# dtee1/reinforcement-learning-for-playing-tetris-with-prescribed-initial-configuration-and-limited-moves

Hardware: AMD Instinct MI355X
Metric: env-steps/sec (whole node) at 1M parallel 20x10 boards (higher is better)
Workload: dtype u32

## Files before the change

### reinforcement-learning-for-playing-tetris-with-prescribed-initial-configuration-and-limited-moves_amd/csrc/tetris_piclim.hip

```cpp
#include "tpl_internal.h"
#include "tpl_observe.h"
#include "tpl_step.h"

#include <hip/hip_bf16.h>

#include <type_traits>

#include <cstdarg>
#include <cstdio>
#include <cstring>
#include <new>

namespace tpl {

static thread_local char g_err[512] = "";

int fail_msg(int code, const char* fmt, ...) {
    va_list ap;
    va_start(ap, fmt);
    vsnprintf(g_err, sizeof(g_err), fmt, ap);
    va_end(ap);
    return code;
}

static inline size_t align_up(size_t x, size_t a) { return (x + a - 1) / a * a; }
constexpr size_t kPlanePad = 512 * 4;
static inline size_t plane_bytes(int64_t n) { return align_up((size_t)n, kPlanePad) * sizeof(uint4); }
static inline size_t clock_bytes(int64_t n) { return align_up((size_t)n, kPlanePad) / kClockGroup * sizeof(unsigned long long); }
static inline int piece_words(int M) { return M / kWindowStride + 1; }
static inline uint32_t record_stride_shift(int M) {
    const size_t need = 32 + 8 * (size_t)(piece_words(M) - 1);
    uint32_t shift = 6;
    while (((size_t)1 << shift) < need) ++shift;
    return shift;
}
static inline size_t record_stride(int M) { return (size_t)1 << record_stride_shift(M); }

#ifdef TPL_DIAG_CLOCK
#define TPL_STAMP(k) stamp[k] = __builtin_amdgcn_s_memrealtime()
#else
#define TPL_STAMP(k) do { } while (0)
#endif

template <bool kActionForm, bool kAutoReset, int kBpl, int kThreads, typename Obs = void>
__global__ __launch_bounds__(kThreads) void step_kernel(const StepArgs p) {
    constexpr bool kObserve = !std::is_void<Obs>::value;
    static_assert(!kObserve || kBpl == 1, "step-and-observe: one board per lane");
    static_assert((int)sizeof(uint32_t) * kLdsCols * kLdsStride <= obs::kWaveLds, "the column words fit the wave's observation bytes");
    __shared__ ShapeWord s_shape[32];
    __shared__ uint32_t s_stat[4];
    __shared__ uint32_t s_cols[kObserve ? 1 : kThreads / 64][kObserve ? 1 : kLdsCols][kObserve ? 1 : kLdsStride];
    __shared__ __attribute__((aligned(16))) uint8_t s_rows[kObserve ? kThreads / 64 : 1][kObserve ? obs::kWaveLds : 16];
#ifdef TPL_DIAG_CLOCK
    unsigned long long stamp[6] = {0, 0, 0, 0, 0, 0};
#endif
    TPL_STAMP(0);

    const int64_t base = (int64_t)blockIdx.x * (kThreads * kBpl) + threadIdx.x;
    uint4 A[kBpl], B[kBpl];
    uint32_t a0[kBpl], a1[kBpl];
    unsigned long long clock[kBpl];
    bool valid[kBpl];
#pragma unroll
    for (int k = 0; k < kBpl; ++k) {
        const int64_t i = base + (int64_t)k * kThreads;
        valid[k] = i < p.n;
        const int64_t j = valid[k] ? i : p.n - 1;
        A[k] = p.plane_a[i];
        B[k] = p.plane_b[i];
        const int64_t wave_first = (int64_t)blockIdx.x * (kThreads * kBpl) + (int64_t)k * kThreads +
                                   (int64_t)(__builtin_amdgcn_readfirstlane((int)threadIdx.x) & ~63);
        clock[k] = p.clock[wave_first >> kClockShift];
        a0[k] = load_int<true>(p.act0, p.int_shift, j);
        a1[k] = kActionForm ? 0u : load_int<true>(p.act1, p.int_shift, j);
    }
    if (threadIdx.x < 32) s_shape[threadIdx.x] = kShapeTable[threadIdx.x];
    if (threadIdx.x < 4) s_stat[threadIdx.x] = 0;
    __syncthreads();

    uint64_t word[kBpl];
    uint32_t moves[kBpl], refill_word[kBpl];
    bool live[kBpl], refill[kBpl];
#pragma unroll
    for (int k = 0; k < kBpl; ++k) {
        asm volatile("" ::"v"(A[k].x), "v"(B[k].x), "v"(a0[k]), "v"(a1[k]), "s"(clock[k]));
    }
    TPL_STAMP(1);
    __builtin_amdgcn_s_setprio(3);
#pragma unroll
    for (int k = 0; k < kBpl; ++k) {
        moves[k] = packed_moves(A[k]);
        const uint32_t tenth = tenths(moves[k] + 1u);
        refill_word[k] = window_word(tenth);
        live[k] = packed_state(B[k]) == ST_RUNNING;
        refill[k] = live[k] && window_runs_out(tenth) && (p.n_cfg[0] | p.n_cfg[1]) != 0u;
    }
#pragma unroll
    for (int k = 0; k < kBpl; ++k) {
        const int64_t i = base + (int64_t)k * kThreads;
        word[k] = 0;
        if (refill[k]) {
            const uint32_t slot = packed_slot(B[k]);
            const uint32_t cfg = config_of(p, (uint32_t)i, clock[k] - moves[k], slot);
            word[k] = piece_word_at(pool_record(p, slot, cfg), refill_word[k]);
        }
    }

    float reward[kBpl];
    uint32_t n_clear[kBpl];
    bool done[kBpl], reload[kBpl];
#pragma unroll
    for (int k = 0; k < kBpl; ++k) {
        reward[k] = 0.0f;
        n_clear[k] = 0;
        done[k] = true;
        reload[k] = false;
        if (!live[k]) continue;
        uint32_t rot, loc;
        if (kActionForm) {
            split_action(a0[k], rot, loc);
        } else {
            rot = a0[k];
            loc = a1[k];
        }
        Board s;
        bool topout;
        unpack_board<true>(A[k], B[k], s);
        uint32_t* cols = kObserve ? (uint32_t*)s_rows[threadIdx.x >> 6] + (threadIdx.x & 63)
                                  : &s_cols[threadIdx.x >> 6][0][threadIdx.x & 63];
        lds_store_cols(cols, s.c);
        if (k == 0) {
#pragma unroll
            for (int c = kCols; c < kLdsCols; ++c) cols[c * kLdsStride] = kSentinelBit;
        }
        n_clear[k] = move_board_lds(s, cols, s_shape, rot, loc, p.L, p.M, topout);
        lds_load_cols(cols, s.c);
        next_window(s, refill[k], word[k]);

        reward[k] = step_reward(p, n_clear[k], s.state);
        done[k] = s.state != ST_RUNNING;
        if (done[k]) {
            atomicAdd(&s_stat[0], 1u);
            if (s.lines) atomicAdd(&s_stat[1], s.lines);
            if (s.state == ST_WON) atomicAdd(&s_stat[2], 1u);
            if (s.state == ST_LOST_TOPOUT) atomicAdd(&s_stat[3], 1u);
        }
        reload[k] = kAutoReset && done[k];
        pack_board<true>(s, A[k], B[k]);
    }

    TPL_STAMP(2);
#pragma unroll
    for (int k = 0; k < kBpl; ++k) {
        const int64_t i = base + (int64_t)k * kThreads;
        if (!valid[k]) continue;
        if (p.reward) p.reward[i] = reward[k];
        if (p.done) p.done[i] = done[k] ? 1 : 0;
        if (p.cleared) p.cleared[i] = (uint8_t)n_clear[k];
    }

    if (kAutoReset) {
        bool any = false;
#pragma unroll
        for (int k = 0; k < kBpl; ++k) any = any || reload[k];
        if (any) {
            uint4 RA[kBpl], RB[kBpl];
#pragma unroll
            for (int k = 0; k < kBpl; ++k) {
                const int64_t i = base + (int64_t)k * kThreads;
                const uint32_t cfg = config_of(p, (uint32_t)i, clock[k] + 1u, p.cur_slot);
                const uint4* rec = (const uint4*)pool_record(p, p.cur_slot, reload[k] ? cfg : 0u);
                RA[k] = rec[0];
                RB[k] = rec[1];
            }
#pragma unroll
            for (int k = 0; k < kBpl; ++k) {
                if (!reload[k]) continue;
                A[k] = RA[k];
                B[k] = make_uint4(RB[k].x, RB[k].y | (p.cur_slot << 30), RB[k].z, RB[k].w);
            }
        }
    }

#ifdef TPL_DIAG_CLOCK
#pragma unroll
    for (int k = 0; k < kBpl; ++k) asm volatile("" ::"v"(A[k].x), "v"(B[k].x));
#endif
    TPL_STAMP(3);
#pragma unroll
    for (int k = 0; k < kBpl; ++k) {
        const int64_t i = base + (int64_t)k * kThreads;
        if (!kAutoReset && !live[k]) continue;
        p.plane_a[i] = A[k];
        p.plane_b[i] = B[k];
    }
    if constexpr (kBpl % 2 == 0) {
        static_assert(kBpl == 2 || kBpl == 4, "one call of store_pair per two boards of a lane");
        const int lane = threadIdx.x & 63;
        const int64_t group_first = (int64_t)blockIdx.x * (kThreads * kBpl) + (threadIdx.x & ~63) + ((lane >> 4) & 1) * kClockGroup;
        const auto store_pair = [&](int k, unsigned long long even, unsigned long long odd) {
            const int64_t i = group_first + (int64_t)(k + (lane >> 5)) * kThreads;
            p.clock[i >> kClockShift] = (lane >> 5 ? odd : even) + 1u;
        };
        store_pair(0, clock[0], clock[1]);
        if constexpr (kBpl == 4) store_pair(2, clock[2], clock[3]);
    } else {
#pragma unroll
        for (int k = 0; k < kBpl; ++k) {
            const int64_t i = base + (int64_t)k * kThreads;
            p.clock[i >> kClockShift] = clock[k] + 1u;
        }
    }

    TPL_STAMP(4);
    if constexpr (kObserve) {
        const int lane = threadIdx.x & 63;
        const int64_t wave_base = (int64_t)blockIdx.x * kThreads + (threadIdx.x & ~63);
        const int64_t left = p.n - wave_base;
        const int count = left >= 64 ? 64 : left > 0 ? (int)left : 0;
        uint8_t* const rows = s_rows[threadIdx.x >> 6];
        int lines_left = 0;
        if (lane < count) {
            Board s;
            unpack_board(A[0], B[0], s);
            lines_left = obs::board_to_bytes(s, p.L, p.M, rows, lane);
        }
        if (count > 0) obs::store_span<Obs>(rows, lane, count, wave_base, lines_left, (Obs*)p.obs);
    }
    __syncthreads();
    if (s_stat[0] != 0) {
        if (threadIdx.x < 4) {
            const uint32_t v = s_stat[threadIdx.x];
            if (v) atomicAdd(&p.stats[(size_t)(blockIdx.x % kStatShards) * kStatStride + threadIdx.x],
                             (unsigned long long)v);
        }
    }
#ifdef TPL_DIAG_CLOCK
    __builtin_amdgcn_s_waitcnt(0);
    TPL_STAMP(5);
    if (p.diag && (threadIdx.x & 63) == 0) {
        unsigned long long* d = p.diag + 6 * ((size_t)blockIdx.x * (kThreads / 64) + (threadIdx.x >> 6));
        for (int k = 0; k < 6; ++k) d[k] = stamp[k];
    }
#endif
}

struct RolloutArgs {
    StepArgs s;
    const uint8_t* actions;
    uint64_t random_seed;
    uint32_t step0;
    uint8_t* actions_out;
    int64_t action_stride;
    uint32_t K;
    float* reward_steps;
    uint8_t* done_steps;
    float* reward_sum;
    uint32_t* finished;
    uint32_t* trajectory;
};

template <bool kAutoReset, bool kRandom, bool kCompact>
__global__ __launch_bounds__(kBlock) void rollout_kernel(const RolloutArgs q) {
    const StepArgs& p = q.s;
    __shared__ ShapeWord s_shape[32];
    __shared__ uint32_t s_stat[4];
    __shared__ uint32_t s_cols[kBlock / 64][kLdsCols][kLdsStride];
    const int64_t i = (int64_t)blockIdx.x * kBlock + threadIdx.x;
    const bool valid = i < p.n;
    uint4 A = make_uint4(0, 0, 0, 0), B = A;
    uint32_t act = 0;
    unsigned long long clock = 0;
    if (valid) {
        A = p.plane_a[i];
        B = p.plane_b[i];
        if (!kRandom) act = q.actions[i];
    }
    const int64_t wave_first = (int64_t)blockIdx.x * kBlock + (int64_t)(__builtin_amdgcn_readfirstlane((int)threadIdx.x) & ~63);
    if (wave_first < p.n) clock = p.clock[wave_first >> kClockShift];
    if (threadIdx.x < 32) s_shape[threadIdx.x] = kShapeTable[threadIdx.x];
    if (threadIdx.x < 4) s_stat[threadIdx.x] = 0;
    __syncthreads();

    RareTally tally;
    if (valid) {
        Board s;
        unpack_board<true>(A, B, s);
        uint32_t* cols = &s_cols[threadIdx.x >> 6][0][threadIdx.x & 63];
        lds_store_cols(cols, s.c);
#pragma unroll
        for (int k = kCols; k < kLdsCols; ++k) cols[k * kLdsStride] = kSentinelBit;
        const uint8_t* next_word = next_piece_word(current_record(s, p, (uint32_t)i, clock), s.moves);
        uint32_t until_refill = moves_until_refill(s.moves);
        const uint32_t draw_base = kRandom ? explore_base(q.random_seed, (uint64_t)(p.global_offset + i)) : 0u;
        uint32_t draw_pair = 0;
        float rsum = 0.0f;
        const int64_t block_first = (int64_t)blockIdx.x * kBlock;
        const uint32_t in_block = threadIdx.x;
        const uint8_t* act_row = q.actions + block_first;
        uint8_t* act_out_row = q.actions_out + block_first;
        float* reward_row = q.reward_steps + block_first;
        uint8_t* done_row = q.done_steps + block_first;
        const bool want_reward = !kCompact && q.reward_steps != nullptr, want_done = !kCompact && q.done_steps != nullptr;
        uint32_t* traj_row = q.trajectory + block_first;
        uint32_t traj_word = 0;
        asm volatile("" ::"v"(act));
        float reward_prev = 0.0f;
        bool done_prev = false;
        for (uint32_t k = 0; k < q.K; ++k) {
            if (!kCompact && k > 0) {
                if (want_reward) { __builtin_nontemporal_store(reward_prev, reward_row + in_block); reward_row += p.n; }
                if (want_done) { __builtin_nontemporal_store((uint8_t)(done_prev ? 1 : 0), done_row + in_block); done_row += p.n; }
            }
            if (kCompact && k > 0 && (k & 3u) == 0u) {
                __builtin_nontemporal_store(traj_word, traj_row + in_block);
                traj_row += p.n;
                traj_word = 0;
            }
            uint32_t act_next = 0;
            if (kRandom) {
                const uint32_t step = q.step0 + k;
                if (k == 0 || (step & 1u) == 0u) draw_pair = explore_pair(draw_base, q.random_seed, step);
                act = explore_pick(draw_pair, step);
                if (q.actions_out) { act_out_row[in_block] = (uint8_t)act; act_out_row += p.n; }
            } else {
                act_row += q.action_stride;
                if (k + 1 < q.K) act_next = act_row[in_block];
            }
            uint32_t rot, loc;
            split_small_action(act, rot, loc);
            float reward;
            uint32_t code;
            const bool done = advance_board_lds<kAutoReset>(s, cols, next_word, until_refill, rot, loc, p, (uint32_t)i, clock + k,
                                                            s_shape, reward, code, tally);
            if (kCompact) traj_word |= code << (8u * (k & 3u));
            else {
                rsum = rsum + reward;
                reward_prev = reward;
                done_prev = done;
            }
            act = act_next;
        }
        if (want_reward) __builtin_nontemporal_store(reward_prev, reward_row + in_block);
        if (want_done) __builtin_nontemporal_store((uint8_t)(done_prev ? 1 : 0), done_row + in_block);
        if (kCompact) __builtin_nontemporal_store(traj_word, traj_row + in_block);
        lds_load_cols(cols, s.c);
        pack_board<true>(s, A, B);
        p.plane_a[i] = A;
        p.plane_b[i] = B;
        if ((threadIdx.x & (kClockGroup - 1)) == 0) p.clock[i >> kClockShift] = clock + q.K;
        if (!kCompact && q.reward_sum) q.reward_sum[i] = rsum;
        if (q.finished) q.finished[i] = tally.episodes;
    }
    flush_tally(tally, s_stat, p.stats);
}

__global__ __launch_bounds__(kBlock) void reset_kernel(const StepArgs p, const uint8_t* mask) {
    const int64_t i = (int64_t)blockIdx.x * kBlock + threadIdx.x;
    if (i >= p.n) return;
    unsigned long long birth = 0;
    if (mask) {
        if (!mask[i]) return;
        birth = p.clock[i >> kClockShift];
    }
    const uint32_t cfg = config_of(p, (uint32_t)i, birth, p.cur_slot);
    uint4 A, B;
    load_config(p, cfg, A, B);
    p.plane_a[i] = A;
    p.plane_b[i] = B;
}

__device__ __forceinline__ uint64_t piece_word(const uint8_t* pc, uint32_t M, uint32_t w) {
    uint64_t word = 0;
    for (uint32_t j = 0; j < (uint32_t)kWindowEntries; ++j) {
        const uint32_t idx = w * kWindowStride + j;
        word |= (uint64_t)(idx <= M ? (uint32_t)(pc[idx] & 7u) : 7u) << (3u * j);
    }
    return word;
}

__global__ __launch_bounds__(kBlock) void pack_configs_kernel(const uint16_t* rows, const uint8_t* pieces, int64_t n_cfg,
                                                             uint32_t M, uint32_t words, uint8_t* pool, uint32_t stride) {
    const int64_t i = (int64_t)blockIdx.x * kBlock + threadIdx.x;
    if (i >= n_cfg) return;
    uint16_t r[kRows];
#pragma unroll
    for (int k = 0; k < kRows; ++k) r[k] = rows[i * kRows + k];
    Board s;
    rows_to_cols(r, s.c);
    const uint8_t* pc = pieces + (size_t)i * (M + 1);
    set_window(s, piece_word(pc, M, 0));
    s.state = ST_RUNNING; s.lines = 0; s.moves = 0; s.slot = 0;
    uint4 A, B;
    pack_board(s, A, B);
    uint8_t* rec = pool + (size_t)i * stride;
    ((uint4*)rec)[0] = A;
    ((uint4*)rec)[1] = B;
    for (uint32_t w = 1; w < words; ++w) ((uint64_t*)(rec + 32))[w - 1] = piece_word(pc, M, w);
}

__global__ __launch_bounds__(kBlock) void build_side_kernel(const uint8_t* pool, uint32_t stride_shift, int64_t n_cfg, uint8_t* side) {
    const int64_t i = (int64_t)blockIdx.x * kBlock + threadIdx.x;
    if (i >= n_cfg) return;
    const uint4* rec = (const uint4*)(pool + ((size_t)i << stride_shift));
    Board s;
    unpack_board<true>(rec[0], rec[1], s);
    uint4* sr = (uint4*)(side + ((size_t)i << kSideShift));
    sr[0] = make_uint4(s.c[0], s.c[1], s.c[2], s.c[3]);
    sr[1] = make_uint4(s.c[4], s.c[5], s.c[6], s.c[7]);
    sr[2] = make_uint4(s.c[8], s.c[9], s.window, s.window_hi);
    sr[3] = make_uint4(0, 0, 0, 0);
}

__global__ __launch_bounds__(kBlock) void export_kernel(const uint4* plane_a, const uint4* plane_b, int64_t n, uint32_t M,
                                                       uint16_t* rows, uint8_t* cur, uint8_t* nxt, uint8_t* lines,
                                                       uint8_t* moves, uint8_t* state, uint8_t* pieces_left) {
    const int64_t i = (int64_t)blockIdx.x * kBlock + threadIdx.x;
    if (i >= n) return;
    Board s;
    unpack_board(plane_a[i], plane_b[i], s);
    if (rows) {
#pragma unroll
        for (int r = 0; r < kRows; ++r) rows[i * kRows + r] = (uint16_t)row_of_cols(s.c, r);
    }
    if (cur) cur[i] = (uint8_t)(s.window & 7u);
    if (nxt) nxt[i] = (uint8_t)((s.window >> 3) & 7u);
    if (lines) lines[i] = (uint8_t)s.lines;
    if (moves) moves[i] = (uint8_t)s.moves;
    if (state) state[i] = (uint8_t)(s.state == ST_LOST_TOPOUT ? ST_LOST_LIMIT : s.state);
    if (pieces_left) pieces_left[i] = (uint8_t)(M + 1u - s.moves - (s.state == ST_LOST_TOPOUT ? 1u : 0u));
}

template <typename T>
__device__ __forceinline__ T obs_cast(float v);
template <> __device__ __forceinline__ float obs_cast<float>(float v) { return v; }
template <> __device__ __forceinline__ __hip_bfloat16 obs_cast<__hip_bfloat16>(float v) { return __float2bfloat16(v); }

template <typename T>
__global__ __launch_bounds__(kBlock) void expand_obs_kernel(const uint4* plane_a, const uint4* plane_b, int64_t n,
                                                           uint32_t L, uint32_t M, T* out) {
    __shared__ uint32_t s_bits[kBlock / 64][64][9];
    const int lane = threadIdx.x & 63;
    const int wave = threadIdx.x >> 6;
    const int64_t base = ((int64_t)blockIdx.x * (kBlock / 64) + wave) * 64;
    const int64_t i = base + lane;
    if (i < n) {
        Board s;
        unpack_board(plane_a[i], plane_b[i], s);
        uint32_t words[7] = {0, 0, 0, 0, 0, 0, 0};
#pragma unroll
        for (int r = 0; r < kRows; ++r) {
            const uint32_t row = row_of_cols(s.c, r);
            const int bit = r * 10;
            words[bit >> 5] |= row << (bit & 31);
            if ((bit & 31) > 22) words[(bit >> 5) + 1] |= row >> (32 - (bit & 31));
        }
#pragma unroll
        for (int k = 0; k < 7; ++k) s_bits[wave][lane][k] = words[k];
        const uint32_t terminal = s.state != ST_RUNNING ? 1u : 0u;
        s_bits[wave][lane][7] = (s.window & 63u) | (terminal << 6) | (s.lines << 8) | (s.moves << 16);
    }
    __syncthreads();
    const int64_t count = (n - base) < 64 ? (n - base) : 64;
    for (int64_t j = 0; j < count; ++j) {
        const uint32_t* bits = s_bits[wave][j];
        T* o = out + (base + j) * TPL_OBS_DIM;
        const uint32_t f = bits[7];
#pragma unroll
        for (int t = 0; t < 4; ++t) {
            const int e = lane + 64 * t;
            if (e < 200) {
                o[e] = obs_cast<T>((float)((bits[e >> 5] >> (e & 31)) & 1u));
            } else if (e < TPL_OBS_DIM) {
                float v;
                if (e < 207) v = ((f & 7u) == (uint32_t)(e - 200)) ? 1.0f : 0.0f;
                else if (e < 214) v = (((f >> 3) & 7u) == (uint32_t)(e - 207)) ? 1.0f : 0.0f;
                else if (e == 214) v = (float)((int)L - (int)((f >> 8) & 0xFFu));
                else if (e == 215) v = (float)((int)M - (int)((f >> 16) & 0xFFu));
                else v = (float)((f >> 6) & 1u);
                o[e] = obs_cast<T>(v);
            }
        }
// ... 670 lines not shown
```

### reinforcement-learning-for-playing-tetris-with-prescribed-initial-configuration-and-limited-moves_amd/csrc/tpl_device.h

```cpp
#pragma once

#include <hip/hip_runtime.h>
#include <stdint.h>

namespace tpl {

constexpr int kRows = 20;
constexpr int kCols = 10;
constexpr uint32_t kColMask = 0xFFFFFu;
constexpr int kWindowStride = 10;
constexpr int kWindowEntries = 12;
constexpr int kSideShift = 6;
constexpr int kClockGroup = 32;
constexpr int kClockShift = 5;

enum : uint32_t { ST_RUNNING = 0, ST_WON = 1, ST_LOST_LIMIT = 2, ST_LOST_TOPOUT = 3 };

struct Board {
    uint32_t c[kCols];
    uint32_t window;
    uint32_t window_hi;
    uint32_t state, lines, moves, slot;
};

__device__ __forceinline__ void set_window(Board& s, uint64_t word) {
    s.window = (uint32_t)word;
    s.window_hi = (uint32_t)(word >> 32) & 0xFu;
}
__device__ __forceinline__ void next_window(Board& s, bool refill, uint64_t word) {
    const uint32_t lo = __builtin_amdgcn_alignbit(s.window_hi, s.window, 3);
    const uint32_t hi = s.window_hi >> 3;
    s.window = refill ? (uint32_t)word : lo;
    s.window_hi = refill ? ((uint32_t)(word >> 32) & 0xFu) : hi;
}
__device__ __forceinline__ uint32_t tenths(uint32_t cursor) { return __umul24(cursor, 205u); }
__device__ __forceinline__ bool window_runs_out(uint32_t t) { return (t & 2047u) < 205u; }
__device__ __forceinline__ uint32_t window_word(uint32_t t) { return t >> 11; }

struct ShapeWord { uint32_t x, y; };

__host__ __device__ constexpr ShapeWord make_shape(int h, int w, int m0, int m1, int m2, int m3,
                                                   int t0, int t1, int t2, int t3) {
    const int m[4] = {m0, m1, m2, m3};
    const int t[4] = {t0, t1, t2, t3};
    uint32_t x = 0, y = 0;
    for (int c = 0; c < 4; ++c) {
        uint32_t colbits = 0;
        for (int i = 0; i < 4; ++i) colbits |= (uint32_t)((m[i] >> c) & 1) << i;
        x |= colbits << (4 * c);
        y |= (uint32_t)(c < w ? 3 - t[c] : 64) << (8 * c);
    }
    x |= (uint32_t)w << 16 | (uint32_t)h << 19 | (uint32_t)(kCols - w) << 22 | ((1u << h) - 1u) << 26;
    return ShapeWord{x, y};
}

#define TPL_I0 make_shape(1, 4, 15, 0, 0, 0, 0, 0, 0, 0)
#define TPL_I1 make_shape(4, 1, 1, 1, 1, 1, 3, 0, 0, 0)
#define TPL_L0 make_shape(2, 3, 4, 7, 0, 0, 1, 1, 1, 0)
#define TPL_L1 make_shape(3, 2, 3, 2, 2, 0, 0, 2, 0, 0)
#define TPL_L2 make_shape(2, 3, 7, 1, 0, 0, 1, 0, 0, 0)
#define TPL_L3 make_shape(3, 2, 1, 1, 3, 0, 2, 2, 0, 0)
#define TPL_J0 make_shape(2, 3, 1, 7, 0, 0, 1, 1, 1, 0)
#define TPL_J1 make_shape(3, 2, 2, 2, 3, 0, 2, 2, 0, 0)
#define TPL_J2 make_shape(2, 3, 7, 4, 0, 0, 0, 0, 1, 0)
#define TPL_J3 make_shape(3, 2, 3, 1, 1, 0, 2, 0, 0, 0)
#define TPL_T0 make_shape(2, 3, 2, 7, 0, 0, 1, 1, 1, 0)
#define TPL_T1 make_shape(3, 2, 2, 3, 2, 0, 1, 2, 0, 0)
#define TPL_T2 make_shape(2, 3, 7, 2, 0, 0, 0, 1, 0, 0)
#define TPL_T3 make_shape(3, 2, 1, 3, 1, 0, 2, 1, 0, 0)
#define TPL_S0 make_shape(2, 3, 6, 3, 0, 0, 1, 1, 0, 0)
#define TPL_S1 make_shape(3, 2, 1, 3, 2, 0, 1, 2, 0, 0)
#define TPL_Z0 make_shape(2, 3, 3, 6, 0, 0, 0, 1, 1, 0)
#define TPL_Z1 make_shape(3, 2, 2, 3, 1, 0, 2, 1, 0, 0)
#define TPL_O0 make_shape(2, 2, 3, 3, 0, 0, 1, 1, 0, 0)

#define TPL_SHAPE_LIST                                                                                    \
    TPL_I0, TPL_I1, TPL_I0, TPL_I1, TPL_L0, TPL_L1, TPL_L2, TPL_L3, TPL_J0, TPL_J1, TPL_J2, TPL_J3, TPL_T0,  \
    TPL_T1, TPL_T2, TPL_T3, TPL_S0, TPL_S1, TPL_S0, TPL_S1, TPL_Z0, TPL_Z1, TPL_Z0, TPL_Z1, TPL_O0, TPL_O0,  \
    TPL_O0, TPL_O0, TPL_O0, TPL_O0, TPL_O0, TPL_O0
__device__ __constant__ const ShapeWord kShapeTable[32] = {TPL_SHAPE_LIST};
constexpr ShapeWord kShapeTableHost[32] = {TPL_SHAPE_LIST};

__device__ __forceinline__ void pack3(uint32_t a, uint32_t b, uint32_t c, uint32_t& lo, uint32_t& hi) {
    lo = a | (b << 20);
    hi = (b >> 12) | (c << 8);
}

constexpr uint32_t kSentinelBit = 1u << kRows;

__device__ __forceinline__ uint32_t opaque_sgpr(uint32_t v) {
    uint32_t r;
    asm("s_mov_b32 %0, %1" : "=s"(r) : "i"(v));
    return r;
}

template <bool kSentinel>
__device__ __forceinline__ void unpack3(uint32_t lo, uint32_t hi, uint32_t& a, uint32_t& b, uint32_t& c) {
    if (kSentinel) {
        const uint32_t m = opaque_sgpr(kColMask), top = opaque_sgpr(kSentinelBit);
        a = (m & lo) | (~m & top);
        b = (m & __builtin_amdgcn_alignbit(hi, lo, 20)) | (~m & top);
        c = (m & (hi >> 8)) | (~m & top);
    } else {
        a = lo & kColMask;
        b = __builtin_amdgcn_alignbit(hi, lo, 20) & kColMask;
        c = (hi >> 8) & kColMask;
    }
}

template <bool kSentinel = false>
__device__ __forceinline__ void unpack_board(const uint4& A, const uint4& B, Board& s) {
    unpack3<kSentinel>(A.x, A.y, s.c[0], s.c[1], s.c[2]);
    unpack3<kSentinel>(A.z, A.w, s.c[3], s.c[4], s.c[5]);
    unpack3<kSentinel>(B.x, B.y, s.c[6], s.c[7], s.c[8]);
    if (kSentinel) {
        const uint32_t m = opaque_sgpr(kColMask), top = opaque_sgpr(kSentinelBit);
        s.c[9] = (m & B.z) | (~m & top);
    } else {
        s.c[9] = B.z & kColMask;
    }
    s.lines = (B.z >> 20) & 0xFFu;
    s.moves = (A.y >> 28) | ((A.w >> 28) << 4);
    s.window = B.w;
    s.window_hi = B.z >> 28;
    s.state = (B.y >> 28) & 3u;
    s.slot = (B.y >> 30) & 1u;
}

__device__ __forceinline__ uint32_t packed_state(const uint4& B) { return (B.y >> 28) & 3u; }
__device__ __forceinline__ uint32_t packed_slot(const uint4& B) { return (B.y >> 30) & 1u; }
__device__ __forceinline__ uint32_t packed_moves(const uint4& A) { return (A.y >> 28) | ((A.w >> 28) << 4); }

template <bool kSentinel = false>
__device__ __forceinline__ void pack_board(const Board& s, uint4& A, uint4& B) {
    uint32_t c[kCols];
#pragma unroll
    for (int k = 0; k < kCols; ++k) c[k] = kSentinel ? (s.c[k] & kColMask) : s.c[k];
    pack3(c[0], c[1], c[2], A.x, A.y);
    pack3(c[3], c[4], c[5], A.z, A.w);
    pack3(c[6], c[7], c[8], B.x, B.y);
    A.y |= s.moves << 28;
    A.w |= (s.moves >> 4) << 28;
    B.y |= (s.state << 28) | (s.slot << 30);
    B.z = c[9] | (s.lines << 20) | (s.window_hi << 28);
    B.w = s.window;
}

__device__ __forceinline__ void rows_to_cols(const uint16_t* rows, uint32_t* c) {
#pragma unroll
    for (int x = 0; x < kCols; ++x) c[x] = 0;
#pragma unroll
    for (int r = 0; r < kRows; ++r) {
        uint32_t v = rows[r];
#pragma unroll
        for (int x = 0; x < kCols; ++x) c[x] |= ((v >> x) & 1u) << r;
    }
}

__device__ __forceinline__ uint32_t row_of_cols(const uint32_t* c, int r) {
    uint32_t v = 0;
#pragma unroll
    for (int x = 0; x < kCols; ++x) v |= ((c[x] >> r) & 1u) << x;
    return v;
}

__device__ __forceinline__ uint32_t blend(uint32_t m, uint32_t x, uint32_t y) { return (m & x) | (~m & y); }

__device__ __forceinline__ uint32_t move_board(Board& s, const ShapeWord* shape, uint32_t rot, uint32_t loc,
                                               uint32_t L, uint32_t M, bool& topout) {
    const ShapeWord sh = shape[(s.window & 7u) * 4u + (rot & 3u)];
    const uint32_t w = (sh.x >> 16) & 7u;
    const uint32_t h = (sh.x >> 19) & 7u;

    loc = min(loc, (uint32_t)kCols - w);

    uint32_t t[kCols];
#pragma unroll
    for (int k = 0; k < kCols; ++k) t[k] = (uint32_t)__builtin_ctz(s.c[k] | kSentinelBit);
    uint32_t p0 = t[0] | (t[1] << 8) | (t[2] << 16) | (t[3] << 24);
    uint32_t p1 = t[4] | (t[5] << 8) | (t[6] << 16) | (t[7] << 24);
    uint32_t p2 = t[8] | (t[9] << 8);
    asm volatile("" : "+v"(p0), "+v"(p1), "+v"(p2));
    const uint32_t word = loc >> 2;
    const uint32_t lo = word == 0u ? p0 : word == 1u ? p1 : p2;
    const uint32_t hi = word == 0u ? p1 : word == 1u ? p2 : 0u;
    const uint32_t tops = __builtin_amdgcn_alignbyte(hi, lo, loc & 3u);
    const uint32_t sums = tops + sh.y;
    const uint32_t best = min(min(sums & 0xFFu, (sums >> 8) & 0xFFu), min((sums >> 16) & 0xFFu, sums >> 24));
    const int drop = (int)best - 4;

    topout = drop < 0;
    const uint32_t dshift = topout ? 0u : (uint32_t)drop;

    uint64_t placed = (uint64_t)(sh.x & 0xFFFFu) << (4u * loc);
    if (topout) placed = 0;
    const uint32_t plo = (uint32_t)placed, phi = (uint32_t)(placed >> 32);
#pragma unroll
    for (int k = 0; k < 8; ++k) s.c[k] |= ((plo >> (4 * k)) & 0xFu) << dshift;
    s.c[8] |= (phi & 0xFu) << dshift;
    s.c[9] |= ((phi >> 4) & 0xFu) << dshift;
    s.moves += topout ? 0u : 1u;

    uint32_t full = s.c[0];
#pragma unroll
    for (int k = 1; k < kCols; ++k) full &= s.c[k];
    uint32_t clear = topout ? 0u : (full & (((1u << h) - 1u) << dshift));
    const uint32_t n = (uint32_t)__builtin_popcount(clear);

    while (clear) {
        const uint32_t r = (uint32_t)__builtin_ctz(clear);
        clear &= clear - 1u;
        const uint32_t above = (1u << r) - 1u;
        const uint32_t keep = ~((above << 1) | 1u);
#pragma unroll
        for (int k = 0; k < kCols; ++k) s.c[k] = (s.c[k] & keep) | ((s.c[k] & above) << 1);
    }
    s.lines += n;

    const bool won = !topout && n != 0u && s.lines >= L;
    const bool limit = !topout && !won && s.moves >= M;
    s.state = topout ? ST_LOST_TOPOUT : won ? ST_WON : limit ? ST_LOST_LIMIT : ST_RUNNING;
    return n;
}

constexpr int kLdsCols = kCols + 3;
constexpr int kLdsStride = 64;

__device__ __forceinline__ void lds_store_cols(uint32_t* cols, const uint32_t (&c)[kCols]) {
#pragma unroll
    for (int k = 0; k < kCols; ++k) cols[k * kLdsStride] = c[k];
}
__device__ __forceinline__ void lds_load_cols(const uint32_t* cols, uint32_t (&c)[kCols]) {
#pragma unroll
    for (int k = 0; k < kCols; ++k) c[k] = cols[k * kLdsStride];
}

struct MoveEnd { bool topout, won, limit; };

template <typename AfterDrop>
__device__ __forceinline__ uint32_t move_board_lds(Board& s, uint32_t* cols, const ShapeWord* shape, uint32_t rot, uint32_t loc,
                                                   uint32_t L, uint32_t M, MoveEnd& end, AfterDrop&& after_drop) {
    const ShapeWord sh = shape[(s.window & 7u) * 4u + (rot & 3u)];
    loc = min(loc, (sh.x >> 22) & 15u);

    uint32_t* under = cols + loc * kLdsStride;
    uint32_t c[4];
#pragma unroll
    for (int j = 0; j < 4; ++j) c[j] = under[j * kLdsStride];
    uint32_t best = 0xFFu;
#pragma unroll
    for (int j = 0; j < 4; ++j) best = min(best, (uint32_t)__builtin_ctz(c[j]) + ((sh.y >> (8 * j)) & 0xFFu));
    const int drop = (int)best - 4;
    const bool topout = drop < 0;
    const uint32_t dshift = topout ? 0u : (uint32_t)drop;
    after_drop(topout);

    const uint32_t pattern = topout ? 0u : sh.x;
#pragma unroll
    for (int j = 0; j < 4; ++j) under[j * kLdsStride] = c[j] | (((pattern >> (4 * j)) & 0xFu) << dshift);
    s.moves += topout ? 0u : 1u;

    uint32_t b[kCols];
    lds_load_cols(cols, b);
    uint32_t full = b[0];
#pragma unroll
    for (int k = 1; k < kCols; ++k) full &= b[k];
    uint32_t clear = topout ? 0u : (full & (((sh.x >> 26) & 15u) << dshift));
    const uint32_t n = (uint32_t)__builtin_popcount(clear);

    if (clear) {
        do {
            const uint32_t r = (uint32_t)__builtin_ctz(clear);
            clear &= clear - 1u;
            const uint32_t above = (1u << r) - 1u;
            const uint32_t keep = ~((above << 1) | 1u);
#pragma unroll
            for (int k = 0; k < kCols; ++k) b[k] = (b[k] & keep) | ((b[k] & above) << 1);
        } while (clear);
        lds_store_cols(cols, b);
    }
    s.lines += n;

    end.topout = topout;
    end.won = !topout && n != 0u && s.lines >= L;
    end.limit = !topout && !end.won && s.moves >= M;
    return n;
}

__device__ __forceinline__ uint32_t move_board_lds(Board& s, uint32_t* cols, const ShapeWord* shape, uint32_t rot, uint32_t loc,
                                                   uint32_t L, uint32_t M, MoveEnd& end) {
    return move_board_lds(s, cols, shape, rot, loc, L, M, end, [](bool) {});
}

__device__ __forceinline__ uint32_t move_board_lds(Board& s, uint32_t* cols, const ShapeWord* shape, uint32_t rot, uint32_t loc,
                                                   uint32_t L, uint32_t M, bool& topout) {
    MoveEnd end;
    const uint32_t n = move_board_lds(s, cols, shape, rot, loc, L, M, end);
    topout = end.topout;
    s.state = end.topout ? ST_LOST_TOPOUT : end.won ? ST_WON : end.limit ? ST_LOST_LIMIT : ST_RUNNING;
    return n;
}

__host__ __device__ __forceinline__ uint64_t sm64(uint64_t x) {
    x += 0x9E3779B97F4A7C15ULL;
    x = (x ^ (x >> 30)) * 0xBF58476D1CE4E5B9ULL;
    x = (x ^ (x >> 27)) * 0x94D049BB133111EBULL;
    return x ^ (x >> 31);
}

__host__ __device__ __forceinline__ uint64_t rng_base(uint64_t seed, uint64_t stream, uint64_t index) {
    return sm64(sm64(seed ^ (stream * 0xD1B54A32D192ED03ULL)) ^ index);
}
__host__ __device__ __forceinline__ uint64_t rng_at(uint64_t base, uint64_t counter) { return sm64(base ^ counter); }
__host__ __device__ __forceinline__ uint64_t rng(uint64_t seed, uint64_t stream, uint64_t index, uint64_t counter) {
    return rng_at(rng_base(seed, stream, index), counter);
}
__host__ __device__ __forceinline__ int rng_range(uint64_t draw, int lo, int hi) {
    return lo + (int)(((draw >> 32) * (uint64_t)(hi - lo + 1)) >> 32);
}

__host__ __device__ __forceinline__ uint32_t fmix32(uint32_t h) {
    h ^= h >> 16; h *= 0x85EBCA6Bu; h ^= h >> 13; h *= 0xC2B2AE35u; h ^= h >> 16;
    return h;
}

struct DecisionStream { uint32_t key, stride; };
__host__ __device__ __forceinline__ DecisionStream decision_stream(uint64_t seed, uint64_t index, uint32_t attempt) {
    const uint64_t w = rng(seed, 4, index, attempt);
    return DecisionStream{(uint32_t)w, (uint32_t)(w >> 32) | 1u};
}
__host__ __device__ __forceinline__ uint32_t decision_word(DecisionStream& s) {
    const uint32_t w = fmix32(s.key);
    s.key += s.stride;
    return w;
}
__host__ __device__ __forceinline__ int word_bag_index(uint32_t w, int n_bag) {
#ifdef __HIP_DEVICE_COMPILE__
    return (int)(__umul24(w >> 20, (uint32_t)n_bag) >> 12);
#else
    return (int)(((w >> 20) * (uint32_t)n_bag) >> 12);
#endif
}
__host__ __device__ __forceinline__ int word_rotations(uint32_t w) { return (int)((w >> 18) & 3u); }
__host__ __device__ __forceinline__ int word_location(uint32_t w, int places) { return (int)(((w & 0x3FFFFu) * (uint32_t)places) >> 18); }

__host__ __device__ __forceinline__ int decision(DecisionStream& s, int lo, int hi) {
    const uint32_t d = fmix32(s.key) >> 8;
    s.key += s.stride;
#ifdef __HIP_DEVICE_COMPILE__
    return lo + (int)(__umul24(d, (uint32_t)(hi - lo + 1)) >> 24);
#else
    return lo + (int)((d * (uint32_t)(hi - lo + 1)) >> 24);
#endif
}

constexpr int kCarveAttempts = 24;
constexpr int kCarveDoublings = 8;
constexpr int64_t kCarveCutoffMax = (int64_t)1 << 28;
__host__ __device__ __forceinline__ int64_t carve_cutoff(int L, int64_t cutoff, int attempt) {
    int64_t c = cutoff;
    if (c <= 0) {
        switch (L) {
            case 1: case 2: case 3: c = 64; break;
            case 4: c = 128; break;     case 5: c = 256; break;     case 6: c = 384; break;     case 7: c = 512; break;
            case 8: c = 768; break;     case 9: c = 1792; break;    case 10: c = 3328; break;   case 11: c = 5376; break;
            case 12: c = 9216; break;   case 13: c = 17408; break;  case 14: c = 36000; break;  case 15: c = 64000; break;
            default: c = 132000; break;
        }
    }
    const int64_t grown = c << (attempt < 12 ? 0 : attempt - 11 < kCarveDoublings ? attempt - 11 : kCarveDoublings);
    return grown < kCarveCutoffMax ? grown : kCarveCutoffMax;
}
__host__ __device__ __forceinline__ int carve_fewest_pieces(int L) { return (L + 1) / 2; }

__host__ __device__ __forceinline__ uint32_t assign_seed(uint64_t seed) { return (uint32_t)(sm64(seed) >> 32); }

__device__ __forceinline__ uint32_t assign_config(int64_t global_offset, uint32_t offset_mod, uint32_t i, uint64_t birth,
                                                  uint32_t seed_mix, uint32_t n_cfg, int mode) {
    if (mode == 1) {
        uint64_t t = (uint64_t)offset_mod + (uint64_t)(i % n_cfg);
        if (t >= n_cfg) t -= n_cfg;
        t += (uint32_t)birth % n_cfg;
        if (t >= n_cfg) t -= n_cfg;
        return (uint32_t)t;
    }
    const uint64_t g = (uint64_t)global_offset + i;
    const uint32_t x = ((uint32_t)g + (uint32_t)birth * 0x9E3779B1u) ^ __umul24((uint32_t)(g >> 32), 0x85EBCBu) ^
                       __umul24((uint32_t)(birth >> 32), 0xC2B2AFu) ^ seed_mix;
    return __umulhi(fmix32(x), n_cfg);
}

}
```

Baseline: 69.61 billion.

## Defer piece-window refill gather to post-move phase merged with auto-reset load

Moves the global gather of the next piece-window word, used when a board's window runs out, from before the move simulation to after it. It now shares one load loop with the auto-reset record fetch, and the word is patched straight into the packed board. The aim is to take a dependent global load off the critical path ahead of the LDS move work and to merge two scattered gathers into one phase. The cost is that the reset branch is now entered for refill-only lanes as well, and the refill load latency is exposed after the move instead of being hidden behind it.

```diff
diff --git a/reinforcement-learning-for-playing-tetris-with-prescribed-initial-configuration-and-limited-moves_amd/csrc/tetris_piclim.hip b/reinforcement-learning-for-playing-tetris-with-prescribed-initial-configuration-and-limited-moves_amd/csrc/tetris_piclim.hip
--- a/reinforcement-learning-for-playing-tetris-with-prescribed-initial-configuration-and-limited-moves_amd/csrc/tetris_piclim.hip
+++ b/reinforcement-learning-for-playing-tetris-with-prescribed-initial-configuration-and-limited-moves_amd/csrc/tetris_piclim.hip
@@ -78,8 +78,7 @@
     if (threadIdx.x < 4) s_stat[threadIdx.x] = 0;
     __syncthreads();
 
-    uint64_t word[kBpl];
-    uint32_t moves[kBpl], refill_word[kBpl];
+    uint32_t moves[kBpl];
     bool live[kBpl], refill[kBpl];
 #pragma unroll
     for (int k = 0; k < kBpl; ++k) {
@@ -90,32 +89,14 @@
 #pragma unroll
     for (int k = 0; k < kBpl; ++k) {
         moves[k] = packed_moves(A[k]);
-        const uint32_t tenth = tenths(moves[k] + 1u);
-        refill_word[k] = window_word(tenth);
         live[k] = packed_state(B[k]) == ST_RUNNING;
-        refill[k] = live[k] && window_runs_out(tenth) && (p.n_cfg[0] | p.n_cfg[1]) != 0u;
-    }
-#pragma unroll
-    for (int k = 0; k < kBpl; ++k) {
-        const int64_t i = base + (int64_t)k * kThreads;
-        word[k] = 0;
-        if (refill[k]) {
-            const uint32_t slot = packed_slot(B[k]);
-            const uint32_t cfg = config_of(p, (uint32_t)i, clock[k] - moves[k], slot);
-            word[k] = piece_word_at(pool_record(p, slot, cfg), refill_word[k]);
-        }
+        refill[k] = live[k] && window_runs_out(tenths(moves[k] + 1u)) && (p.n_cfg[0] | p.n_cfg[1]) != 0u;
     }
 
     float reward[kBpl];
     uint32_t n_clear[kBpl];
     bool done[kBpl], reload[kBpl];
-#pragma unroll
-    for (int k = 0; k < kBpl; ++k) {
-        reward[k] = 0.0f;
-        n_clear[k] = 0;
-        done[k] = true;
-        reload[k] = false;
-        if (!live[k]) continue;
+    const auto move_one = [&](int k) {
         uint32_t rot, loc;
         if (kActionForm) {
             split_action(a0[k], rot, loc);
@@ -135,7 +116,7 @@
         }
         n_clear[k] = move_board_lds(s, cols, s_shape, rot, loc, p.L, p.M, topout);
         lds_load_cols(cols, s.c);
-        next_window(s, refill[k], word[k]);
+        pop_window(s);
 
         reward[k] = step_reward(p, n_clear[k], s.state);
         done[k] = s.state != ST_RUNNING;
@@ -147,6 +128,14 @@
         }
         reload[k] = kAutoReset && done[k];
         pack_board<true>(s, A[k], B[k]);
+    };
+#pragma unroll
+    for (int k = 0; k < kBpl; ++k) {
+        reward[k] = 0.0f;
+        n_clear[k] = 0;
+        done[k] = true;
+        reload[k] = false;
+        if (live[k]) move_one(k);
     }
 
     TPL_STAMP(2);
@@ -159,25 +148,35 @@
         if (p.cleared) p.cleared[i] = (uint8_t)n_clear[k];
     }
 
-    if (kAutoReset) {
-        bool any = false;
-#pragma unroll
-        for (int k = 0; k < kBpl; ++k) any = any || reload[k];
+    {
+        bool patch[kBpl], any = false;
+#pragma unroll
+        for (int k = 0; k < kBpl; ++k) {
+            patch[k] = refill[k] && !reload[k];
+            any = any || reload[k] || patch[k];
+        }
         if (any) {
-            uint4 RA[kBpl], RB[kBpl];
+            uint64_t word[kBpl];
 #pragma unroll
             for (int k = 0; k < kBpl; ++k) {
                 const int64_t i = base + (int64_t)k * kThreads;
-                const uint32_t cfg = config_of(p, (uint32_t)i, clock[k] + 1u, p.cur_slot);
-                const uint4* rec = (const uint4*)pool_record(p, p.cur_slot, reload[k] ? cfg : 0u);
-                RA[k] = rec[0];
-                RB[k] = rec[1];
+                const uint32_t slot = patch[k] ? packed_slot(B[k]) : p.cur_slot;
+                const uint64_t birth = clock[k] + (patch[k] ? 0ull - (uint64_t)moves[k] : 1ull);
+                const uint8_t* rec = pool_record(p, slot, config_of(p, (uint32_t)i, birth, slot));
+                asm volatile("" : "=v"(word[k]));
+                if (reload[k]) {
+                    A[k] = ((const uint4*)rec)[0];
+                    B[k] = ((const uint4*)rec)[1];
+                } else if (patch[k]) {
+                    word[k] = piece_word_at(rec, window_word(tenths(moves[k] + 1u)));
+                }
             }
 #pragma unroll
+            for (int k = 0; k < kBpl; ++k) asm volatile("" ::"v"(word[k]), "v"(A[k].x), "v"(B[k].x));
+#pragma unroll
             for (int k = 0; k < kBpl; ++k) {
-                if (!reload[k]) continue;
-                A[k] = RA[k];
-                B[k] = make_uint4(RB[k].x, RB[k].y | (p.cur_slot << 30), RB[k].z, RB[k].w);
+                if (patch[k]) patch_window(B[k], word[k]);
+                if (reload[k]) B[k].y |= p.cur_slot << 30;
             }
         }
     }
diff --git a/reinforcement-learning-for-playing-tetris-with-prescribed-initial-configuration-and-limited-moves_amd/csrc/tpl_device.h b/reinforcement-learning-for-playing-tetris-with-prescribed-initial-configuration-and-limited-moves_amd/csrc/tpl_device.h
--- a/reinforcement-learning-for-playing-tetris-with-prescribed-initial-configuration-and-limited-moves_amd/csrc/tpl_device.h
+++ b/reinforcement-learning-for-playing-tetris-with-prescribed-initial-configuration-and-limited-moves_amd/csrc/tpl_device.h
@@ -32,6 +32,10 @@
     const uint32_t hi = s.window_hi >> 3;
     s.window = refill ? (uint32_t)word : lo;
     s.window_hi = refill ? ((uint32_t)(word >> 32) & 0xFu) : hi;
+}
+__device__ __forceinline__ void pop_window(Board& s) {
+    s.window = __builtin_amdgcn_alignbit(s.window_hi, s.window, 3);
+    s.window_hi >>= 3;
 }
 __device__ __forceinline__ uint32_t tenths(uint32_t cursor) { return __umul24(cursor, 205u); }
 __device__ __forceinline__ bool window_runs_out(uint32_t t) { return (t & 2047u) < 205u; }
@@ -145,6 +149,10 @@
     B.z = c[9] | (s.lines << 20) | (s.window_hi << 28);
     B.w = s.window;
 }
+__device__ __forceinline__ void patch_window(uint4& B, uint64_t word) {
+    B.w = (uint32_t)word;
+    B.z = (B.z & 0x0FFFFFFFu) | ((uint32_t)(word >> 32) << 28);
+}
 
 __device__ __forceinline__ void rows_to_cols(const uint16_t* rows, uint32_t* c) {
 #pragma unroll
```

Result: faster. 70.38 billion, median of 6 (+1.1%).
